# DreamWaterFound/self_commit_ORB-SLAM2

Measured on AMD Instinct MI355X. Metric: frames/s ORB extract+match (1000 feat, 640x480), higher is better.
Workload: dtype u8; 1 GPU; batch of 256 synthetic 640x480 frames per GPU (8 distinct resident batches per step, one launch set per batch), ORB extract (1000 feat, 8 levels, FAST 20/7) + brute-force Hamming SearchByBoW of consecutive frames; batch_per_gpu=256, streams=3, width=640, height=480, nfeatures=1000, parallelism=frames sharded, 1 rank(s), no data-path collective

## Files before the change

### self_commit_orb-slam2_amd/csrc/orbx_match.hip

```cpp
#include <math.h>
#include <string.h>

#include <atomic>
#include <chrono>

#include <type_traits>
#include <vector>

#include "orbx_match_internal.h"

using namespace orbx_match;

namespace {

__global__ __launch_bounds__(256) void k_bow_order(FeatDev A, const int32_t *__restrict__ pairsA, int32_t *__restrict__ order, int stride)
{
    const int p = blockIdx.y, fa = pairsA[p];
    const int nA = min(A.counts[fa], A.cap);
    const int i = blockIdx.x * 256 + threadIdx.x;
    if (i >= nA) return;
    int32_t *ord = order + (size_t)p * stride;
    if (!A.groups) { ord[i] = i; return; }
    const int32_t *g = A.groups + (size_t)fa * A.cap;
    const int gi = g[i];
// ... 387 lines not shown
    const bool act = live && !(FILTER && gA < 0);
#pragma unroll
    for (int q = 0; q < TOPK; q++) kk[q] = act ? sentinel : 0u;
    uint32_t th = kk[TOPK - 1] >> 16;
    __syncthreads();
    const unsigned char *myB = sDesc + (size_t)sl * slicePitch;
    const int j0 = sl * per, jn = max(0, min(per, nB - j0));
    for (int j = 0; j < per; j++) {
        const uint4 lo = *(const uint4 *)(myB + (size_t)j * 32), hi = *(const uint4 *)(myB + (size_t)j * 32 + 16);
        uint32_t d = bcnt_acc(a[0] ^ lo.x, 0u);
        d = bcnt_acc(a[1] ^ lo.y, d); d = bcnt_acc(a[2] ^ lo.z, d); d = bcnt_acc(a[3] ^ lo.w, d);
        d = bcnt_acc(a[4] ^ hi.x, d); d = bcnt_acc(a[5] ^ hi.y, d); d = bcnt_acc(a[6] ^ hi.z, d); d = bcnt_acc(a[7] ^ hi.w, d);
        if (FILTER) d = sG[j0 + j] == gA ? d : 0xffffu;
        const uint32_t key = (j < jn && d < th) ? (d << 16) | (uint32_t)(j0 + j) : 0xffffffffu;
        if (__any(key < kk[TOPK - 1])) { topk_insert(kk, key); th = kk[TOPK - 1] >> 16; }
    }
#pragma unroll
    for (int m = 1; m < PAIR_SLICES; m <<= 1) {
        uint32_t other[TOPK];
#pragma unroll
        for (int q = 0; q < TOPK; q++) other[q] = (uint32_t)__shfl_xor((int)kk[q], m);
#pragma unroll
        for (int q = 0; q < TOPK; q++) if (__any(other[q] < kk[TOPK - 1])) topk_insert(kk, other[q]);
    }
    if (sl == 0 && live) {
        uint4 *out = (uint4 *)(topk + (size_t)row * TOPK);
        uint32_t o[TOPK];
#pragma unroll
        for (int q = 0; q < TOPK; q++) o[q] = (!act || kk[q] >= sentinel) ? KEY_EMPTY : kk[q];
        out[0] = make_uint4(o[0], o[1], o[2], o[3]); out[1] = make_uint4(o[4], o[5], o[6], o[7]);
    }
}

#define GREEDY_THREADS 1024
__global__ __launch_bounds__(GREEDY_THREADS) void k_bow_greedy(FeatDev A, FeatDev B, const int32_t *__restrict__ pairsA, const int32_t *__restrict__ pairsB, int mode,
                                                    float nnratio, int checkOri, const uint32_t *__restrict__ topk, const int32_t *__restrict__ order,
                                                    int32_t *__restrict__ matches, int32_t *__restrict__ dists, int32_t *__restrict__ nmatches, int stride, TriDev T,
                                                    int32_t *__restrict__ pubMatches, unsigned long long *pubFlag, unsigned long long pubSeq)
{
    extern __shared__ __attribute__((aligned(16))) unsigned char smem[];
    __shared__ int hist[HISTO_LENGTH];
    __shared__ int sChangedP[2], sQueued, sTotal, sRemoved;
    const int p = blockIdx.x, tid = threadIdx.x, lane = tid & 63, wv = tid >> 6, fa = pairsA[p], fb = pairsB[p];
    const int nA = min(A.counts[fa], A.cap), nB = min(B.counts[fb], B.cap);
    uint32_t *owner = (uint32_t *)smem;
    uint32_t *dec = owner + B.cap;
    unsigned short *sOrd = (unsigned short *)(dec + A.cap);
    unsigned short *queue = sOrd + ((A.cap + 7) & ~7);
    float *sAngB = pubFlag ? (float *)(queue + ((A.cap + 7) & ~7)) : nullptr;
    int32_t *sRes = pubFlag ? (int32_t *)(sAngB + B.cap) : nullptr;
    int32_t *mout = matches + (size_t)p * stride, *dout = dists + (size_t)p * stride;
    const uint4 *tk = (const uint4 *)(topk + (size_t)p * stride * TOPK);
    const orbx_keypoint *kA = A.kp + (size_t)fa * A.cap, *kB = B.kp + (size_t)fb * B.cap;
    if (tid < HISTO_LENGTH) hist[tid] = 0;
    if (tid == 0) { sTotal = 0; sRemoved = 0; }
    float angA0 = 0.0f;
    {
        const int32_t *ord = order + (size_t)p * stride;
        for (int r = tid; r < nA; r += GREEDY_THREADS) {
            int i = ord[r];
            if (pubFlag && r == tid) angA0 = kA[i].angle;
            if (A.valid && !A.valid[(size_t)fa * A.cap + i]) i = 0xffff;
            sOrd[r] = (unsigned short)i;
            dec[r] = KEY_EMPTY;
        }
    }
    if (pubFlag) {
        for (int j = tid; j < nB; j += GREEDY_THREADS) sAngB[j] = kB[j].angle;
        const int nOut0 = mode == 0 ? nB : nA;
        for (int s2 = tid; s2 < nOut0; s2 += GREEDY_THREADS) sRes[s2] = -1;
    }
    for (int s = tid; s < stride; s += GREEDY_THREADS) { mout[s] = -1; dout[s] = 256; }
    uint4 myK0 = make_uint4(0u, 0u, 0u, 0u), myK1 = myK0, othK0 = myK0, othK1 = myK0;
    bool haveKeys = false;
    for (int j = tid; j < nB; j += GREEDY_THREADS) owner[j] = 0xffffffffu;
    if (tid == 0) { sChangedP[0] = 0; sChangedP[1] = 0; sQueued = 0; }
    for (int par = 0;; par ^= 1) {
        __syncthreads();
        for (int r = tid; r < nA; r += GREEDY_THREADS) {
            const uint32_t d = dec[r];
            if (d != KEY_EMPTY) atomicMin(&owner[d & 0xffff], (uint32_t)r);
        }
        __syncthreads();
        bool changed = false;
        for (int r = tid; r < nA; r += GREEDY_THREADS) {
            const int i = sOrd[r];
            if (i == 0xffff) continue;
            if (r != tid || !haveKeys) { const uint4 q0 = tk[i * 2], q1 = tk[i * 2 + 1]; if (r == tid) { myK0 = q0; myK1 = q1; haveKeys = true; } else { othK0 = q0; othK1 = q1; } }
            const uint4 q0 = r == tid ? myK0 : othK0, q1 = r == tid ? myK1 : othK1;
            const uint32_t keys[TOPK] = {q0.x, q0.y, q0.z, q0.w, q1.x, q1.y, q1.z, q1.w};
            auto half = [&](const int k0, uint32_t &h1, uint32_t &h2) -> int {
                uint32_t bi[4], ow[4];
#pragma unroll
                for (int k = 0; k < 4; k++) {
                    const uint32_t low = keys[k0 + k] & 0xffffu;
                    bi[k] = keys[k0 + k] == KEY_EMPTY ? 0u : (mode == 2 ? 0xffffu - low : low);
                }
#pragma unroll
                for (int k = 0; k < 4; k++) ow[k] = owner[bi[k]];
                int nf = 0;
                h1 = KEY_EMPTY; h2 = KEY_EMPTY;
#pragma unroll
                for (int k = 3; k >= 0; k--) {
                    const bool fr = keys[k0 + k] != KEY_EMPTY && ow[k] >= (uint32_t)r;
                    const uint32_t packed = (keys[k0 + k] & 0xffff0000u) | bi[k];
                    h2 = fr ? h1 : h2;
                    h1 = fr ? packed : h1;
                    nf += fr ? 1 : 0;
                }
                return nf;
            };
            uint32_t k1, k2;
            int nfree = half(0, k1, k2);
            if (nfree < 2 && (keys[4] & keys[5] & keys[6] & keys[7]) != KEY_EMPTY) {
                uint32_t j1, j2;
                const int nb = half(4, j1, j2);
                k2 = nfree == 1 ? j1 : j2;
                k1 = nfree == 1 ? k1 : j1;
                nfree += nb;
            }
            const uint32_t bestKey = k1;
            const int best2 = nfree >= 2 ? (int)(k2 >> 16) : 256;
            if (nfree < (mode == 2 ? 1 : 2) && keys[TOPK - 1] != KEY_EMPTY) { queue[atomicAdd(&sQueued, 1)] = (unsigned short)r; continue; }
            uint32_t nd = KEY_EMPTY;
            if (bestKey != KEY_EMPTY) {
                const int best1 = (int)(bestKey >> 16);
                if (mode == 2) nd = bestKey;
                else {
                    const bool pass = mode == 0 ? (best1 <= TH_LOW) : (best1 < TH_LOW);
                    if (pass && (float)best1 < nnratio * (float)best2) nd = bestKey;
                }
            }
            if (nd != dec[r]) { dec[r] = nd; changed = true; }
        }
        if (changed) sChangedP[par] = 1;
        __syncthreads();
        const int nq = sQueued;
        for (int q = wv; q < nq; q += GREEDY_THREADS / 64) {
            const int r = queue[q], i = sOrd[r];
            const unsigned long long *da = (const unsigned long long *)(A.desc + ((size_t)fa * A.cap + i) * 32);
            unsigned long long a[4] = {da[0], da[1], da[2], da[3]};
            const int gA = A.groups ? A.groups[(size_t)fa * A.cap + i] : 0;
            uint32_t k0 = KEY_EMPTY, k1 = KEY_EMPTY;
            for (int jj = lane; jj < nB; jj += 64) {
                if (owner[jj] < (uint32_t)r) continue;
                if (B.groups && B.groups[(size_t)fb * B.cap + jj] != gA) continue;
                if (mode >= 1 && B.valid && !B.valid[(size_t)fb * B.cap + jj]) continue;
                const unsigned long long *db = (const unsigned long long *)(B.desc + ((size_t)fb * B.cap + jj) * 32);
                int d = hamming256(a, db[0], db[1], db[2], db[3]);
                uint32_t kk = ((uint32_t)d << 16) | (uint32_t)jj;
                if (mode == 2) {
                    if (d > TH_LOW) continue;
                    const size_t ia = (size_t)fa * A.cap + i;
                    if (!tri_geom_ok(T, p, A.kp[ia], T.stereoA && T.stereoA[ia], B.kp[(size_t)fb * B.cap + jj], T.stereoB && T.stereoB[(size_t)fb * B.cap + jj])) continue;
                    kk = ((uint32_t)d << 16) | (0xffffu - (uint32_t)jj);
                }
                if (kk < k0) { k1 = k0; k0 = kk; } else if (kk < k1) k1 = kk;
            }
            uint32_t bestKey = wave_min(k0);
            if (k0 == bestKey) k0 = k1;
            const uint32_t second = wave_min(k0);
            uint32_t nd = KEY_EMPTY;
            if (bestKey != KEY_EMPTY) {
                const int best1 = (int)(bestKey >> 16), best2 = second != KEY_EMPTY ? (int)(second >> 16) : 256;
                if (mode == 2) nd = (bestKey & 0xffff0000u) | (0xffffu - (bestKey & 0xffffu));
                else {
                    const bool pass = mode == 0 ? (best1 <= TH_LOW) : (best1 < TH_LOW);
                    if (pass && (float)best1 < nnratio * (float)best2) nd = bestKey;
                }
            }
            if (lane == 0 && nd != dec[r]) { dec[r] = nd; sChangedP[par] = 1; }
        }
        if (nq) __syncthreads();
        const int again = sChangedP[par];
        if (!again) break;
        for (int j = tid; j < nB; j += GREEDY_THREADS) owner[j] = 0xffffffffu;
        if (tid == 0) { sChangedP[par ^ 1] = 0; sQueued = 0; }
    }
    const float factor = HISTO_LENGTH / 360.0f;
    int total = 0;
    for (int r = tid; r < nA; r += GREEDY_THREADS) {
        const uint32_t d = dec[r];
        if (d == KEY_EMPTY) continue;
        const int i = sOrd[r], bj = (int)(d & 0xffff), slot = mode == 0 ? bj : i;
        mout[slot] = mode == 0 ? i : bj; dout[slot] = (int)(d >> 16);
        if (sRes) sRes[slot] = mode == 0 ? i : bj;
        total++;
        if (checkOri) {
            float rot = ((pubFlag && r == tid) ? angA0 : kA[i].angle) - (sAngB ? sAngB[bj] : kB[bj].angle);
            if (rot < 0.0f) rot += 360.0f;
            int bin = (int)roundf(rot * factor);
            if (bin == HISTO_LENGTH) bin = 0;
            dec[r] = d | ((uint32_t)bin << 26);
            atomicAdd(&hist[bin], 1);
        }
    }
    total = wave_sum_xor(total);
    if (lane == 0 && total) atomicAdd(&sTotal, total);
    __syncthreads();
    if (checkOri) {
        int ind1, ind2, ind3;
        three_maxima_wave(hist, lane, ind1, ind2, ind3);
        int removed = 0;
        for (int r = tid; r < nA; r += GREEDY_THREADS) {
            const uint32_t d = dec[r];
            if (d == KEY_EMPTY) continue;
            const int b = (int)(d >> 26);
            if (b != ind1 && b != ind2 && b != ind3) {
                const int slot = mode == 0 ? (int)(d & 0xffff) : (int)sOrd[r];
                mout[slot] = -1; dout[slot] = 256; removed++;
                if (sRes) sRes[slot] = -1;
            }
        }
        removed = wave_sum_xor(removed);
        if (lane == 0 && removed) atomicAdd(&sRemoved, removed);
    }
    __syncthreads();
    if (tid == 0) nmatches[p] = sTotal - sRemoved;
    if (pubFlag) {
        const int nOut = mode == 0 ? nB : nA;
        for (int s2 = tid; s2 < nOut; s2 += GREEDY_THREADS) pubMatches[s2] = sRes[s2];
        if (tid == 0) pubMatches[nOut] = sTotal - sRemoved;
        orbx_publish(nullptr, pubFlag, pubSeq, 1u);
    }
}

__global__ __launch_bounds__(256) void k_stereo(FeatDev Lf, FeatDev Rf, const int32_t *__restrict__ pairsL, const int32_t *__restrict__ pairsR,
                                                const float *__restrict__ scaleFactors, float maxD, int32_t *__restrict__ bestIdx, int32_t *__restrict__ bestDist,
                                                int32_t *__restrict__ nmatches, int stride)
{
    const int p = blockIdx.y, fl = pairsL[p], fr = pairsR[p];
    const int nL = min(Lf.counts[fl], Lf.cap), nR = min(Rf.counts[fr], Rf.cap);
    const int lane = threadIdx.x & 63, iL = blockIdx.x * 4 + (threadIdx.x >> 6);
    if (iL >= nL) return;
    const orbx_keypoint kl = Lf.kp[(size_t)fl * Lf.cap + iL];
    const int row = (int)kl.y;
    const float minU = kl.x - maxD, maxU = kl.x - 0.0f;
    const unsigned long long *da = (const unsigned long long *)(Lf.desc + ((size_t)fl * Lf.cap + iL) * 32);
    unsigned long long a[4] = {da[0], da[1], da[2], da[3]};
    uint32_t best = ((uint32_t)TH_HIGH << 16);
    if (!(maxU < 0)) {
        const orbx_keypoint *kr = Rf.kp + (size_t)fr * Rf.cap;
        for (int iR = lane; iR < nR; iR += 64) {
            const orbx_keypoint k = kr[iR];
            const float r = 2.0f * scaleFactors[k.octave];
            const int maxr = (int)ceilf(k.y + r), minr = (int)floorf(k.y - r);
            if (row < minr || row > maxr) continue;
            if (k.octave < kl.octave - 1 || k.octave > kl.octave + 1) continue;
            if (!(k.x >= minU && k.x <= maxU)) continue;
            const unsigned long long *db = (const unsigned long long *)(Rf.desc + ((size_t)fr * Rf.cap + iR) * 32);
            const int d = hamming256(a, db[0], db[1], db[2], db[3]);
            const uint32_t key = ((uint32_t)d << 16) | (uint32_t)iR;
            if (d < TH_HIGH && key < best) best = key;
        }
// ... 373 lines not shown
        dist += __builtin_popcountll(x ^ y);
    }
    return dist;
}

extern "C" int orbx_matcher_create(int device, int max_features, int max_pairs, orbx_matcher **out)
{
    if (!out || max_features < 1 || max_features > 65535 || max_pairs < 1) { orbx_set_error("bad matcher arguments (1 <= max_features <= 65535)"); return ORBX_ERR_ARG; }
    *out = nullptr;
    orbx_matcher *m = new orbx_matcher();
    m->maxFeatures = max_features; m->maxPairs = max_pairs;
    int rc = m->open(device);
    hipEvent_t *const sync[] = {&m->evDep, &m->evDep2, &m->evPyr[0], &m->evPyr[1], &m->evDone[0], &m->evDone[1]};
    for (hipEvent_t *e : sync) if (!rc) rc = orbx_event_create(e, hipEventDisableTiming);
    for (int r = 0; r < MATCH_PROF_RING; r++)
        for (hipEvent_t *e : {&m->ev0[r], &m->ev1[r], &m->evMid[r]}) if (!rc) rc = orbx_event_create(e);
    const size_t S = (size_t)max_features, P = (size_t)max_pairs;
    if (rc || (rc = m->pairsA.ensure(P)) || (rc = m->pairsB.ensure(P)) || (rc = m->order.ensure(P * S)) || (rc = m->matches.ensure(P * S)) ||
        (rc = m->dists.ensure(P * S)) || (rc = m->nmatches.ensure(P)) || (rc = m->topk.ensure(P * S * TOPK)) || (rc = m->scales.ensure(128)) ||
        (rc = m->uright.ensure(P * S)) || (rc = m->depth.ensure(P * S)) || (rc = m->sad.ensure(P * S))) {
        orbx_matcher_destroy(m);
        return rc;
    }
    *out = m;
    return ORBX_OK;
}

extern "C" void orbx_matcher_destroy(orbx_matcher *m) { orbx_destroy_handle(m); }

__global__ void k_status_or(int *dst, const int *src, int first) { if (first) *dst = *src; else if (*src) atomicOr(dst, *src); }

namespace orbx_match {

int inherit_status(orbx_matcher *m, orbx_extractor *after, bool first)
{
    if (!after) return ORBX_OK;
    const int *w = orbx_extractor_status_word_internal(after);
    if (!w) return ORBX_OK;
    if (!m->producerStatus.p) {
        int rc = m->producerStatus.ensure(1);
        if (rc != ORBX_OK) return rc;
        ORBX_HIP_CHECK(hipMemsetAsync(m->producerStatus.p, 0, sizeof(int), m->stream));
    }
    hipLaunchKernelGGL(k_status_or, dim3(1), dim3(1), 0, m->stream, m->producerStatus.p, w, first ? 1 : 0);
    return ORBX_OK;
}

int check_producer_status(orbx_matcher *m)
{
    if (!m->producerStatus.p) return ORBX_OK;
    int v = 0;
    ORBX_HIP_CHECK(hipMemcpy(&v, m->producerStatus.p, sizeof(int), hipMemcpyDeviceToHost));
    if (!v) return ORBX_OK;
    ORBX_HIP_CHECK(hipMemset(m->producerStatus.p, 0, sizeof(int)));
    orbx_set_error("the extractor batch these results were computed from overflowed a device capacity (bits 0x%x: 1 = >%d FAST candidates in a level, "
                   "2 = quadtree node list, 4 = level keypoints): results are not the reference's", v, 32768);
    return ORBX_ERR_CAPACITY;
}

int prep_pairs(orbx_matcher *m, const orbx_feature_set *a, const orbx_feature_set *b, const int32_t *pa, const int32_t *pb, int npairs,
                      orbx_extractor *after)
{
    if (!m || !a || !b || !pa || !pb) { orbx_set_error("NULL argument"); return ORBX_ERR_ARG; }
    if (npairs < 1 || npairs > m->maxPairs) { orbx_set_error("npairs %d outside 1..%d", npairs, m->maxPairs); return ORBX_ERR_CAPACITY; }
    if (a->capacity > m->maxFeatures || b->capacity > m->maxFeatures || a->capacity < 1 || b->capacity < 1) {
        orbx_set_error("feature capacity %d/%d exceeds the matcher's max_features %d", a->capacity, b->capacity, m->maxFeatures);
        return ORBX_ERR_CAPACITY;
    }
    if (!a->keypoints || !a->descriptors || !a->counts || !b->keypoints || !b->descriptors || !b->counts) { orbx_set_error("NULL feature arrays"); return ORBX_ERR_ARG; }
    for (int p = 0; p < npairs; p++)
        if (pa[p] < 0 || pa[p] >= a->nframes || pb[p] < 0 || pb[p] >= b->nframes) { orbx_set_error("pair %d references a frame out of range", p); return ORBX_ERR_ARG; }
    ORBX_HIP_CHECK(hipSetDevice(m->device));
    if (after) {
        ORBX_HIP_CHECK(hipEventRecord(m->evDep, orbx_extractor_stream_internal(after)));
        ORBX_HIP_CHECK(hipStreamWaitEvent(m->stream, m->evDep, 0));
        int rcs = inherit_status(m, after, true);
        if (rcs != ORBX_OK) return rcs;
    } else if (m->producerStatus.p)
        ORBX_HIP_CHECK(hipMemsetAsync(m->producerStatus.p, 0, sizeof(int), m->stream));
    ORBX_HIP_CHECK(hipMemcpyAsync(m->pairsA.p, pa, (size_t)npairs * sizeof(int32_t), hipMemcpyHostToDevice, m->stream));
    ORBX_HIP_CHECK(hipMemcpyAsync(m->pairsB.p, pb, (size_t)npairs * sizeof(int32_t), hipMemcpyHostToDevice, m->stream));
    return ORBX_OK;
}

int chain_back(orbx_matcher *m, orbx_extractor *after)
{
    if (!after) return ORBX_OK;
    hipEvent_t ev = m->evDone[m->doneSlot];
    m->doneSlot ^= 1;
    ORBX_HIP_CHECK(hipEventRecord(ev, m->stream));
    orbx_extractor_set_consumer_event_internal(after, ev);
    return ORBX_OK;
}

FeatDev to_dev(const orbx_feature_set *s)
{
    FeatDev f;
    f.kp = s->keypoints; f.desc = s->descriptors; f.counts = s->counts; f.groups = s->groups; f.valid = s->valid; f.cap = s->capacity;
    return f;
}

}

extern "C" int orbx_search_by_bow_device(orbx_matcher *m, const orbx_feature_set *a, const orbx_feature_set *b, const int32_t *pairs_a,
                                         const int32_t *pairs_b, int npairs, const orbx_bow_params *params, orbx_extractor *after)
{
    if (!params || (params->mode != 0 && params->mode != 1)) { orbx_set_error("bad bow params"); return ORBX_ERR_ARG; }
    int rc = prep_pairs(m, a, b, pairs_a, pairs_b, npairs, after);
    if (rc != ORBX_OK) return rc;
    const int stride = m->maxFeatures;
    FeatDev A = to_dev(a), B = to_dev(b);
    const int slot = m->profCount % MATCH_PROF_RING;
    ORBX_HIP_CHECK(hipEventRecord(m->ev0[slot], m->stream));
    uint32_t dcut = TH_LOW + 1;
    while (dcut < 257 && !(params->nn_ratio * (float)dcut > (float)TH_LOW)) dcut++;
    const bool filter = b->groups != nullptr || (params->mode == 1 && b->valid != nullptr);
    const dim3 gridTopk((unsigned)((a->capacity + TOPK_ROWS - 1) / TOPK_ROWS), (unsigned)npairs);
    if (filter)
        hipLaunchKernelGGL((k_bow_topk<true, false, TOPK_NROW>), gridTopk, dim3(256), 0, m->stream, A, B, m->pairsA.p, m->pairsB.p, params->mode, dcut, m->topk.p, stride, TriDev());
    else {
        const char *em = getenv("ORBX_MATCH_MFMA");
        const bool mfma = em && em[0] == '1';
        static const int dbg = getenv("ORBX_MFMA_DEBUG") ? atoi(getenv("ORBX_MFMA_DEBUG")) : 0;
        if (mfma) hipLaunchKernelGGL(k_bow_topk_mfma, dim3((unsigned)((a->capacity + 255) / 256), (unsigned)npairs), dim3(256), 0, m->stream, A, B, m->pairsA.p, m->pairsB.p, dcut, m->topk.p, stride, dbg);
        else hipLaunchKernelGGL((k_bow_topk<false, false, TOPK_NROW>), gridTopk, dim3(256), 0, m->stream, A, B, m->pairsA.p, m->pairsB.p, params->mode, dcut, m->topk.p, stride, TriDev());
    }
    ORBX_LAUNCH_CHECK();
    ORBX_HIP_CHECK(hipEventRecord(m->evMid[slot], m->stream));
    m->midValid[slot] = true;
    hipLaunchKernelGGL(k_bow_order, dim3((unsigned)((a->capacity + 255) / 256), (unsigned)npairs), dim3(256), 0, m->stream, A, m->pairsA.p, m->order.p, stride);
    ORBX_LAUNCH_CHECK();
    const size_t ldsGreedy = (size_t)b->capacity * 4 + (size_t)a->capacity * 4 + (size_t)((a->capacity + 7) & ~7) * 2 * 2;
    if (ldsGreedy > 160 * 1024) { orbx_set_error("feature capacity %d too large for the LDS tile", a->capacity); return ORBX_ERR_CAPACITY; }
    if (ldsGreedy > 48 * 1024) ORBX_HIP_CHECK(hipFuncSetAttribute((const void *)k_bow_greedy, hipFuncAttributeMaxDynamicSharedMemorySize, (int)ldsGreedy));
    hipLaunchKernelGGL(k_bow_greedy, dim3((unsigned)npairs), dim3(GREEDY_THREADS), ldsGreedy, m->stream, A, B, m->pairsA.p, m->pairsB.p, params->mode, params->nn_ratio,
                       params->check_orientation, m->topk.p, m->order.p, m->matches.p, m->dists.p, m->nmatches.p, stride, TriDev(), (int32_t *)nullptr, (unsigned long long *)nullptr, 0ull);
    ORBX_LAUNCH_CHECK();
    ORBX_HIP_CHECK(hipEventRecord(m->ev1[slot], m->stream));
    m->profCount++;
    m->lastPairs = npairs; m->lastStride = stride;
    return chain_back(m, after);
}

extern "C" int orbx_stereo_match_device(orbx_matcher *m, const orbx_feature_set *left, const orbx_feature_set *right, const int32_t *pairs_l,
                                        const int32_t *pairs_r, int npairs, const float *scale_factors, int nlevels, float max_disparity,
                                        orbx_extractor *after)
{
    if (!scale_factors || nlevels < 1 || nlevels > 64) { orbx_set_error("bad scale factor table"); return ORBX_ERR_ARG; }
    int rc = prep_pairs(m, left, right, pairs_l, pairs_r, npairs, after);
    if (rc != ORBX_OK) return rc;
    const int stride = m->maxFeatures;
    ORBX_HIP_CHECK(hipMemcpyAsync(m->scales.p, scale_factors, (size_t)nlevels * sizeof(float), hipMemcpyHostToDevice, m->stream));
    ORBX_HIP_CHECK(hipMemsetAsync(m->nmatches.p, 0, (size_t)npairs * sizeof(int32_t), m->stream));
    const int slot = m->profCount % MATCH_PROF_RING;
    ORBX_HIP_CHECK(hipEventRecord(m->ev0[slot], m->stream));
    m->midValid[slot] = false;
    hipLaunchKernelGGL(k_stereo, dim3((unsigned)((left->capacity + 3) / 4), (unsigned)npairs), dim3(256), 0, m->stream, to_dev(left), to_dev(right), m->pairsA.p,
                       m->pairsB.p, m->scales.p, max_disparity, m->matches.p, m->dists.p, m->nmatches.p, stride);
    ORBX_LAUNCH_CHECK();
    ORBX_HIP_CHECK(hipEventRecord(m->ev1[slot], m->stream));
    m->profCount++;
    m->lastPairs = npairs; m->lastStride = stride;
    return chain_back(m, after);
}

extern "C" int orbx_compute_stereo_matches_device(orbx_matcher *m, orbx_extractor *left, orbx_extractor *right, const int32_t *frames_l,
                                                  const int32_t *frames_r, int npairs, float mbf, float mb)
{
    if (!m || !left || !right || !frames_l || !frames_r) { orbx_set_error("NULL argument"); return ORBX_ERR_ARG; }
    OrbxLastBatchView vl, vr;
// ... 321 lines not shown
    const auto sDescB = pin.add(b->descriptors, NB * 32);
    const auto sGrB = pin.add(b->groups, b->groups ? NB : 0);
    const auto sValB = pin.add(b->valid, b->valid ? NB : 0);
    const auto sCnt = pin.add(cnt, 2);
    const auto rRes = pout.hole<int32_t>((size_t)nOut + 1);
    int rc;
    const OrbxStaged sg = bx.begin(m->stream, &rc);
    if (rc != ORBX_OK) return rc;
    uint8_t *ar;
    if ((rc = orbx_stage_to_arena(bx, m->arena, m->stream, 512, &ar)) != ORBX_OK) return rc;
    ORBX_LAUNCH_CHECK();
    const int32_t *dc = sCnt.in(ar);
    FeatDev A, B;
    A.kp = sKpA.in(ar); A.desc = sDescA.in(ar); A.groups = a->groups ? sGrA.in(ar) : nullptr; A.valid = a->valid ? sValA.in(ar) : nullptr; A.counts = dc; A.cap = nA;
    B.kp = sKpB.in(ar); B.desc = sDescB.in(ar); B.groups = b->groups ? sGrB.in(ar) : nullptr; B.valid = b->valid ? sValB.in(ar) : nullptr; B.counts = dc + 1; B.cap = nB;
    uint32_t dcut = TH_LOW + 1;
    while (dcut < 257 && !(prm->nn_ratio * (float)dcut > (float)TH_LOW)) dcut++;
    const bool filter = b->groups != nullptr || (prm->mode == 1 && b->valid != nullptr);
    const int nRowBlocks = (nA + PAIR_ROWS - 1) / PAIR_ROWS, nOrder = (nA + 31) / 32;
    const int per = (nB + PAIR_SLICES - 1) / PAIR_SLICES;
    const size_t ldsPair = std::max((size_t)PAIR_SLICES * ((size_t)per * 32 + 16) + (size_t)PAIR_SLICES * per * 4, (size_t)4096 * 4);
    if ((rc = m->topk.ensure(NA * TOPK)) != ORBX_OK || (rc = m->order.ensure(NA)) != ORBX_OK) return rc;
    const dim3 grid((unsigned)(nRowBlocks + nOrder));
    if (filter) {
        if (ldsPair > 48 * 1024) ORBX_HIP_CHECK(hipFuncSetAttribute((const void *)k_bow_topk_pair<true>, hipFuncAttributeMaxDynamicSharedMemorySize, (int)ldsPair));
        hipLaunchKernelGGL(k_bow_topk_pair<true>, grid, dim3(256), ldsPair, m->stream, A, B, prm->mode, dcut, nRowBlocks, per, m->topk.p, m->order.p);
    } else {
        if (ldsPair > 48 * 1024) ORBX_HIP_CHECK(hipFuncSetAttribute((const void *)k_bow_topk_pair<false>, hipFuncAttributeMaxDynamicSharedMemorySize, (int)ldsPair));
        hipLaunchKernelGGL(k_bow_topk_pair<false>, grid, dim3(256), ldsPair, m->stream, A, B, prm->mode, dcut, nRowBlocks, per, m->topk.p, m->order.p);
    }
    ORBX_LAUNCH_CHECK();
    const size_t ldsGreedy = NB * 4 + NA * 4 + (size_t)((nA + 7) & ~7) * 2 * 2 + NB * 4 + std::max(NA, NB) * 4;
    if (ldsGreedy > 160 * 1024) { orbx_set_error("feature count %d too large for the LDS tile", nA); return ORBX_ERR_CAPACITY; }
    if (ldsGreedy > 48 * 1024) ORBX_HIP_CHECK(hipFuncSetAttribute((const void *)k_bow_greedy, hipFuncAttributeMaxDynamicSharedMemorySize, (int)ldsGreedy));
    if (!m->sfZero.p) {
        if ((rc = m->sfZero.ensure(4)) != ORBX_OK) return rc;
        ORBX_HIP_CHECK(hipMemsetAsync(m->sfZero.p, 0, 4 * sizeof(int32_t), m->stream));
    }
    const int stride = m->maxFeatures;
    const unsigned long long seq = bx.arm();
    hipLaunchKernelGGL(k_bow_greedy, dim3(1), dim3(GREEDY_THREADS), ldsGreedy, m->stream, A, B, (const int32_t *)m->sfZero.p, (const int32_t *)m->sfZero.p, prm->mode, prm->nn_ratio,
                       prm->check_orientation, m->topk.p, m->order.p, m->matches.p, m->dists.p, m->nmatches.p, stride, TriDev(), sg.dev(rRes), bx.flagDev, seq);
    ORBX_LAUNCH_CHECK();
    m->lastPairs = 1; m->lastStride = stride;
    if ((rc = bx.wait(m->stream)) != ORBX_OK) return rc;
    const int32_t *res = sg.host(rRes);
    if (nOut > 0) memcpy(matches, res, (size_t)nOut * 4);
    *nmatches = res[nOut];
    return ORBX_OK;
}

extern "C" int orbx_search_by_bow(orbx_matcher *m, const orbx_feature_set *a_host, const orbx_feature_set *b_host, const orbx_bow_params *params,
                                  int32_t *matches, int32_t *nmatches)
{
    if (!m || !matches || !nmatches) { orbx_set_error("NULL argument"); return ORBX_ERR_ARG; }
    if (!params || (params->mode != 0 && params->mode != 1)) { orbx_set_error("bad bow params"); return ORBX_ERR_ARG; }
    ORBX_HIP_CHECK(hipSetDevice(m->device));
    static const bool split = !(getenv("ORBX_BOW_SINGLE_SPLIT") && getenv("ORBX_BOW_SINGLE_SPLIT")[0] == '0');
    if (split && a_host && b_host && a_host->keypoints && a_host->descriptors && a_host->counts && b_host->keypoints && b_host->descriptors && b_host->counts &&
        a_host->counts[0] > 0 && b_host->counts[0] > 0 && a_host->counts[0] <= m->maxFeatures && b_host->counts[0] <= std::min(m->maxFeatures, 4000))
        return search_by_bow_single(m, a_host, b_host, params, matches, nmatches);
    orbx_feature_set da, db;
    const orbx_feature_set *const hostSets[2] = {a_host, b_host};
    orbx_feature_set *const devSets[2] = {&da, &db};
    int rc;
    if ((rc = stage_host(m, hostSets, devSets, 2)) != ORBX_OK) return rc;
    const int32_t zero = 0;
    if ((rc = orbx_search_by_bow_device(m, &da, &db, &zero, &zero, 1, params, nullptr)) != ORBX_OK) return rc;
    ORBX_HIP_CHECK(hipStreamSynchronize(m->stream));
    const int nOut = params->mode == 0 ? b_host->counts[0] : a_host->counts[0];
    if (nOut > 0) ORBX_HIP_CHECK(hipMemcpy(matches, m->matches.p, (size_t)nOut * 4, hipMemcpyDeviceToHost));
    ORBX_HIP_CHECK(hipMemcpy(nmatches, m->nmatches.p, 4, hipMemcpyDeviceToHost));
    return ORBX_OK;
}

extern "C" int orbx_search_for_triangulation_device(orbx_matcher *m, const orbx_feature_set *a, const orbx_feature_set *b, const int32_t *pairs_a,
                                                    const int32_t *pairs_b, int npairs, const orbx_triangulation_params *params, orbx_extractor *after)
{
    if (!params || !params->f12 || !params->epipole || !params->scale_factors || !params->level_sigma2) { orbx_set_error("bad triangulation params"); return ORBX_ERR_ARG; }
    if (params->nlevels < 1 || params->nlevels > ORBX_MAX_LEVELS) { orbx_set_error("nlevels %d outside 1..%d", params->nlevels, ORBX_MAX_LEVELS); return ORBX_ERR_ARG; }
    int rc = prep_pairs(m, a, b, pairs_a, pairs_b, npairs, after);
    if (rc != ORBX_OK) return rc;
    if ((rc = m->triGeom.ensure((size_t)11 * m->maxPairs)) != ORBX_OK) return rc;
    ORBX_HIP_CHECK(hipMemcpyAsync(m->triGeom.p, params->f12, (size_t)9 * npairs * sizeof(float), hipMemcpyHostToDevice, m->stream));
    ORBX_HIP_CHECK(hipMemcpyAsync(m->triGeom.p + (size_t)9 * m->maxPairs, params->epipole, (size_t)2 * npairs * sizeof(float), hipMemcpyHostToDevice, m->stream));
    TriDev T = TriDev();
    T.f12 = m->triGeom.p; T.epipole = m->triGeom.p + (size_t)9 * m->maxPairs;
    T.stereoA = params->stereo_a; T.stereoB = params->stereo_b;
    for (int l = 0; l < params->nlevels; l++) {
        T.epiTh[l] = 100 * params->scale_factors[l];
        T.chiTh[l] = 3.84 * params->level_sigma2[l];
    }
    const int stride = m->maxFeatures;
    FeatDev A = to_dev(a), B = to_dev(b);
    const int slot = m->profCount % MATCH_PROF_RING;
    ORBX_HIP_CHECK(hipEventRecord(m->ev0[slot], m->stream));
    hipLaunchKernelGGL(k_bow_order, dim3((unsigned)((a->capacity + 255) / 256), (unsigned)npairs), dim3(256), 0, m->stream, A, m->pairsA.p, m->order.p, stride);
    ORBX_LAUNCH_CHECK();
    const dim3 gridTopk((unsigned)((a->capacity + TOPK_ROWS - 1) / TOPK_ROWS), (unsigned)npairs);
    hipLaunchKernelGGL((k_bow_topk<true, true, TOPK_NROW>), gridTopk, dim3(256), 0, m->stream, A, B, m->pairsA.p, m->pairsB.p, 2, (uint32_t)(TH_LOW + 1), m->topk.p, stride, T);
    ORBX_LAUNCH_CHECK();
    m->midValid[slot] = false;
    const size_t ldsGreedy = (size_t)b->capacity * 4 + (size_t)a->capacity * 4 + (size_t)((a->capacity + 7) & ~7) * 2 * 2;
    if (ldsGreedy > 160 * 1024) { orbx_set_error("feature capacity %d too large for the LDS tile", a->capacity); return ORBX_ERR_CAPACITY; }
    if (ldsGreedy > 48 * 1024) ORBX_HIP_CHECK(hipFuncSetAttribute((const void *)k_bow_greedy, hipFuncAttributeMaxDynamicSharedMemorySize, (int)ldsGreedy));
    hipLaunchKernelGGL(k_bow_greedy, dim3((unsigned)npairs), dim3(GREEDY_THREADS), ldsGreedy, m->stream, A, B, m->pairsA.p, m->pairsB.p, 2, 0.0f, params->check_orientation,
                       m->topk.p, m->order.p, m->matches.p, m->dists.p, m->nmatches.p, stride, T, (int32_t *)nullptr, (unsigned long long *)nullptr, 0ull);
    ORBX_LAUNCH_CHECK();
    ORBX_HIP_CHECK(hipEventRecord(m->ev1[slot], m->stream));
    m->profCount++;
    m->lastPairs = npairs; m->lastStride = stride;
    return chain_back(m, after);
}

extern "C" int orbx_search_for_triangulation(orbx_matcher *m, const orbx_feature_set *a_host, const orbx_feature_set *b_host,
                                             const orbx_triangulation_params *params_host, int32_t *matches12, int32_t *nmatches)
{
    if (!m || !params_host || !matches12 || !nmatches) { orbx_set_error("NULL argument"); return ORBX_ERR_ARG; }
    ORBX_HIP_CHECK(hipSetDevice(m->device));
    orbx_feature_set da, db;
    const orbx_feature_set *const hostSets[2] = {a_host, b_host};
    orbx_feature_set *const devSets[2] = {&da, &db};
    int rc;
    if ((rc = stage_host(m, hostSets, devSets, 2)) != ORBX_OK) return rc;
    orbx_triangulation_params P = *params_host;
    const uint8_t *hostFlags[2] = {params_host->stereo_a, params_host->stereo_b};
    const int cnt[2] = {a_host->counts[0], b_host->counts[0]};
    const uint8_t *devFlags[2] = {nullptr, nullptr};
    for (int sd = 0; sd < 2; sd++) {
        if (!hostFlags[sd]) continue;
        if ((rc = m->hs[sd].ensure((size_t)m->maxFeatures)) != ORBX_OK) return rc;
        if (cnt[sd] > 0) ORBX_HIP_CHECK(hipMemcpyAsync(m->hs[sd].p, hostFlags[sd], (size_t)cnt[sd], hipMemcpyHostToDevice, m->stream));
        devFlags[sd] = m->hs[sd].p;
    }
    P.stereo_a = devFlags[0]; P.stereo_b = devFlags[1];
    const int32_t zero = 0;
    if ((rc = orbx_search_for_triangulation_device(m, &da, &db, &zero, &zero, 1, &P, nullptr)) != ORBX_OK) return rc;
    ORBX_HIP_CHECK(hipStreamSynchronize(m->stream));
    if (cnt[0] > 0) ORBX_HIP_CHECK(hipMemcpy(matches12, m->matches.p, (size_t)cnt[0] * 4, hipMemcpyDeviceToHost));
    ORBX_HIP_CHECK(hipMemcpy(nmatches, m->nmatches.p, 4, hipMemcpyDeviceToHost));
    return ORBX_OK;
// ... 23 lines not shown
```

### self_commit_orb-slam2_amd/csrc/orbx_match_internal.h

```cpp
#ifndef ORBX_MATCH_INTERNAL_H
#define ORBX_MATCH_INTERNAL_H

#include "orbx_handle.h"
#include <vector>

#define TH_HIGH 100
#define TH_LOW 50
#define HISTO_LENGTH 30
#define KEY_EMPTY 0xffffffffu
#define TOPK 8
#define MATCH_PROF_RING 64

#define KEY64_EMPTY 0xffffffffffffffffull
#define GRID_COLS 64
#define GRID_ROWS 48

struct FeatDev {
    const orbx_keypoint *kp;
    const uint8_t *desc;
    const int32_t *counts;
    const int32_t *groups;
    const uint8_t *valid;
    int cap;
};
// ... 6 lines not shown

__device__ __forceinline__ void three_maxima_wave(const int *hist, int lane, int &ind1, int &ind2, int &ind3)
{
    const int c = lane < HISTO_LENGTH ? hist[lane] : 0;
    uint32_t key = c > 0 ? ((uint32_t)c << 5) | (uint32_t)(31 - lane) : 0u;
    uint32_t top[3];
#pragma unroll
    for (int k = 0; k < 3; k++) {
        uint32_t v = key;
#pragma unroll
        for (int o = 32; o > 0; o >>= 1) { const uint32_t u = __shfl_xor(v, o); v = u > v ? u : v; }
        top[k] = v;
        if (key == v) key = 0u;
    }
    const int max1 = (int)(top[0] >> 5), max2 = (int)(top[1] >> 5), max3 = (int)(top[2] >> 5);
    ind1 = top[0] ? 31 - (int)(top[0] & 31u) : -1; ind2 = top[1] ? 31 - (int)(top[1] & 31u) : -1; ind3 = top[2] ? 31 - (int)(top[2] & 31u) : -1;
    if ((float)max2 < 0.1f * (float)max1) { ind2 = -1; ind3 = -1; }
    else if ((float)max3 < 0.1f * (float)max1) { ind3 = -1; }
}

struct ProjFrameDev { const orbx_keypoint *kp; const uint8_t *desc; const float *uRight; const uint8_t *occupied; const int32_t *counts; int cap;
                      float minX, minY, gwInv, ghInv; };

struct orbx_matcher : OrbxHandle {
    int maxFeatures = 0, maxPairs = 0;
    hipEvent_t evDep = nullptr, evDone[2] = {nullptr, nullptr};
    int doneSlot = 0;
    hipEvent_t ev0[MATCH_PROF_RING] = {}, ev1[MATCH_PROF_RING] = {};
    hipEvent_t evMid[MATCH_PROF_RING] = {};
    bool midValid[MATCH_PROF_RING] = {};
    float lastDistanceMs = 0.f, lastReplayMs = 0.f;
    int profCount = 0;
    OrbxOwnedBuf<int32_t> pairsA, pairsB, order, matches, dists, nmatches;
    OrbxOwnedBuf<uint32_t> topk;
    OrbxOwnedBuf<float> scales, uright, depth, pf[2];
    OrbxOwnedBuf<unsigned long long> topk64;
    OrbxOwnedBuf<uint8_t> pb[2];
    OrbxOwnedBuf<int32_t> pi32[2];
    OrbxOwnedBuf<orbx_keypoint> pkp;
    OrbxOwnedBuf<uint32_t> projDec, projQueue;
    OrbxHostStage hostStage;
    OrbxCallBox box;
    OrbxOwnedBuf<uint8_t> arena;
    OrbxOwnedBuf<int32_t> sad;
    OrbxOwnedBuf<int32_t> stRowStart, stRowList;
    hipEvent_t evDep2 = nullptr, evPyr[2] = {nullptr, nullptr};
    int lastStereoPairs = 0;
    float sfScales[128] = {};
    int sfLevels = 0;
    OrbxOwnedBuf<int32_t> sfZero;
    OrbxOwnedBuf<float> sfScalesDev;
    float *sfHost = nullptr, *sfHostDev = nullptr;
    size_t sfHostFloats = 0;
    int sfSeq = 0, sfFlagSeq = 0;
    int sfPending = 0;
    OrbxOwnedBuf<orbx_keypoint> hk[2];
    OrbxOwnedBuf<uint8_t> hd[2], hv[2];
    OrbxOwnedBuf<int32_t> hc[2], hg[2];
    OrbxOwnedBuf<uint8_t> hs[2];
    OrbxOwnedBuf<float> triGeom;
    OrbxOwnedBuf<float> frProj;
    OrbxOwnedBuf<int32_t> frLevel;
    OrbxOwnedBuf<uint8_t> frInView;
    size_t frCount = 0;
    int lastPairs = 0, lastStride = 0;
    OrbxOwnedBuf<int> producerStatus;
// ... 41 lines not shown
                if (gamma != 0.0) {
                    const double zeta = (beta - alpha) / (2.0 * gamma);
                    const double t = copysign(1.0, zeta) / (fabs(zeta) + sqrt(1.0 + zeta * zeta));
                    c = 1.0 / sqrt(1.0 + t * t);
                    s = c * t;
                }
#pragma unroll
                for (int r = 0; r < 4; r++) {
                    const double ap = a[p][r], aq = a[q][r];
                    a[p][r] = c * ap - s * aq;
                    a[q][r] = s * ap + c * aq;
                    const double vp = v[p][r], vq = v[q][r];
                    v[p][r] = c * vp - s * vq;
                    v[q][r] = s * vp + c * vq;
                }
            }
        }
    }
    double best = 0.0;
#pragma unroll
    for (int c = 0; c < 4; c++) {
        double n2 = 0.0;
#pragma unroll
        for (int r = 0; r < 4; r++) n2 = n2 + a[c][r] * a[c][r];
        const bool take = c == 0 || n2 < best;
        best = take ? n2 : best;
#pragma unroll
        for (int r = 0; r < 4; r++) nv[r] = take ? v[c][r] : nv[r];
    }
}
#endif

namespace orbx_match {
int prep_pairs(orbx_matcher *m, const orbx_feature_set *a, const orbx_feature_set *b, const int32_t *pa, const int32_t *pb, int npairs, orbx_extractor *after);
int chain_back(orbx_matcher *m, orbx_extractor *after);
int inherit_status(orbx_matcher *m, orbx_extractor *after, bool first = true);
int check_producer_status(orbx_matcher *m);
FeatDev to_dev(const orbx_feature_set *s);
int stage_host(orbx_matcher *m, const orbx_feature_set *const *h, orbx_feature_set *const *d, int nsides);
}

#endif
```

Before: 316,900 frames/s.

## Cut BoW matcher launch overhead and keep replay top-k keys in registers

```diff
diff --git a/self_commit_orb-slam2_amd/csrc/orbx_match.hip b/self_commit_orb-slam2_amd/csrc/orbx_match.hip
--- a/self_commit_orb-slam2_amd/csrc/orbx_match.hip
+++ b/self_commit_orb-slam2_amd/csrc/orbx_match.hip
@@ -443,12 +443,16 @@
     }
 }
 
-#define GREEDY_THREADS 1024
-__global__ __launch_bounds__(GREEDY_THREADS) void k_bow_greedy(FeatDev A, FeatDev B, const int32_t *__restrict__ pairsA, const int32_t *__restrict__ pairsB, int mode,
+#define REPLAY_REG_RANKS 1024
+template <int THREADS>
+__global__ __launch_bounds__(THREADS) void k_bow_greedy(FeatDev A, FeatDev B, const int32_t *__restrict__ pairsA, const int32_t *__restrict__ pairsB, int mode,
                                                     float nnratio, int checkOri, const uint32_t *__restrict__ topk, const int32_t *__restrict__ order,
                                                     int32_t *__restrict__ matches, int32_t *__restrict__ dists, int32_t *__restrict__ nmatches, int stride, TriDev T,
-                                                    int32_t *__restrict__ pubMatches, unsigned long long *pubFlag, unsigned long long pubSeq)
-{
+                                                    int32_t *__restrict__ pubMatches, unsigned long long *pubFlag, unsigned long long pubSeq,
+                                                    int *statusDst, const int *statusSrc)
+{
+    static_assert(THREADS >= 64 && THREADS % 64 == 0 && THREADS <= 1024, "whole waves; the histogram is cleared by the first HISTO_LENGTH threads");
+    constexpr int RPT = (REPLAY_REG_RANKS + THREADS - 1) / THREADS;
     extern __shared__ __attribute__((aligned(16))) unsigned char smem[];
     __shared__ int hist[HISTO_LENGTH];
     __shared__ int sChangedP[2], sQueued, sTotal, sRemoved;
@@ -465,40 +469,47 @@
     const orbx_keypoint *kA = A.kp + (size_t)fa * A.cap, *kB = B.kp + (size_t)fb * B.cap;
     if (tid < HISTO_LENGTH) hist[tid] = 0;
     if (tid == 0) { sTotal = 0; sRemoved = 0; }
+    if (statusDst && p == 0 && tid == 0) *statusDst = *statusSrc;
     float angA0 = 0.0f;
+    uint4 myK0[RPT], myK1[RPT];
     {
-        const int32_t *ord = order + (size_t)p * stride;
-        for (int r = tid; r < nA; r += GREEDY_THREADS) {
-            int i = ord[r];
+        const int32_t *ord = order ? order + (size_t)p * stride : nullptr;
+        auto initRank = [&](const int r) -> int {
+            int i = ord ? ord[r] : r;
             if (pubFlag && r == tid) angA0 = kA[i].angle;
             if (A.valid && !A.valid[(size_t)fa * A.cap + i]) i = 0xffff;
             sOrd[r] = (unsigned short)i;
             dec[r] = KEY_EMPTY;
-        }
+            return i;
+        };
+#pragma unroll
+        for (int s = 0; s < RPT; s++) {
+            myK0[s] = make_uint4(0u, 0u, 0u, 0u); myK1[s] = myK0[s];
+            const int r = tid + s * THREADS;
+            if (r < nA) {
+                const int i = initRank(r);
+                if (i != 0xffff) { myK0[s] = tk[i * 2]; myK1[s] = tk[i * 2 + 1]; }
+            }
+        }
+        for (int r = tid + RPT * THREADS; r < nA; r += THREADS) initRank(r);
     }
     if (pubFlag) {
-        for (int j = tid; j < nB; j += GREEDY_THREADS) sAngB[j] = kB[j].angle;
+        for (int j = tid; j < nB; j += THREADS) sAngB[j] = kB[j].angle;
         const int nOut0 = mode == 0 ? nB : nA;
-        for (int s2 = tid; s2 < nOut0; s2 += GREEDY_THREADS) sRes[s2] = -1;
-    }
-    for (int s = tid; s < stride; s += GREEDY_THREADS) { mout[s] = -1; dout[s] = 256; }
-    uint4 myK0 = make_uint4(0u, 0u, 0u, 0u), myK1 = myK0, othK0 = myK0, othK1 = myK0;
-    bool haveKeys = false;
-    for (int j = tid; j < nB; j += GREEDY_THREADS) owner[j] = 0xffffffffu;
+        for (int s2 = tid; s2 < nOut0; s2 += THREADS) sRes[s2] = -1;
+    }
+    for (int s = tid; s < stride; s += THREADS) { mout[s] = -1; dout[s] = 256; }
+    for (int j = tid; j < nB; j += THREADS) owner[j] = 0xffffffffu;
     if (tid == 0) { sChangedP[0] = 0; sChangedP[1] = 0; sQueued = 0; }
     for (int par = 0;; par ^= 1) {
         __syncthreads();
-        for (int r = tid; r < nA; r += GREEDY_THREADS) {
+        for (int r = tid; r < nA; r += THREADS) {
             const uint32_t d = dec[r];
             if (d != KEY_EMPTY) atomicMin(&owner[d & 0xffff], (uint32_t)r);
         }
         __syncthreads();
         bool changed = false;
-        for (int r = tid; r < nA; r += GREEDY_THREADS) {
-            const int i = sOrd[r];
-            if (i == 0xffff) continue;
-            if (r != tid || !haveKeys) { const uint4 q0 = tk[i * 2], q1 = tk[i * 2 + 1]; if (r == tid) { myK0 = q0; myK1 = q1; haveKeys = true; } else { othK0 = q0; othK1 = q1; } }
-            const uint4 q0 = r == tid ? myK0 : othK0, q1 = r == tid ? myK1 : othK1;
+        auto decide = [&](const int r, const uint4 q0, const uint4 q1) {
             const uint32_t keys[TOPK] = {q0.x, q0.y, q0.z, q0.w, q1.x, q1.y, q1.z, q1.w};
             auto half = [&](const int k0, uint32_t &h1, uint32_t &h2) -> int {
                 uint32_t bi[4], ow[4];
@@ -532,7 +543,7 @@
             }
             const uint32_t bestKey = k1;
             const int best2 = nfree >= 2 ? (int)(k2 >> 16) : 256;
-            if (nfree < (mode == 2 ? 1 : 2) && keys[TOPK - 1] != KEY_EMPTY) { queue[atomicAdd(&sQueued, 1)] = (unsigned short)r; continue; }
+            if (nfree < (mode == 2 ? 1 : 2) && keys[TOPK - 1] != KEY_EMPTY) { queue[atomicAdd(&sQueued, 1)] = (unsigned short)r; return; }
             uint32_t nd = KEY_EMPTY;
             if (bestKey != KEY_EMPTY) {
                 const int best1 = (int)(bestKey >> 16);
@@ -543,11 +554,20 @@
                 }
             }
             if (nd != dec[r]) { dec[r] = nd; changed = true; }
+        };
+#pragma unroll
+        for (int s = 0; s < RPT; s++) {
+            const int r = tid + s * THREADS;
+            if (r < nA && sOrd[r] != 0xffff) decide(r, myK0[s], myK1[s]);
+        }
+        for (int r = tid + RPT * THREADS; r < nA; r += THREADS) {
+            const int i = sOrd[r];
+            if (i != 0xffff) decide(r, tk[i * 2], tk[i * 2 + 1]);
         }
         if (changed) sChangedP[par] = 1;
         __syncthreads();
         const int nq = sQueued;
-        for (int q = wv; q < nq; q += GREEDY_THREADS / 64) {
+        for (int q = wv; q < nq; q += THREADS / 64) {
             const int r = queue[q], i = sOrd[r];
             const unsigned long long *da = (const unsigned long long *)(A.desc + ((size_t)fa * A.cap + i) * 32);
             unsigned long long a[4] = {da[0], da[1], da[2], da[3]};
@@ -585,12 +605,12 @@
         if (nq) __syncthreads();
         const int again = sChangedP[par];
         if (!again) break;
-        for (int j = tid; j < nB; j += GREEDY_THREADS) owner[j] = 0xffffffffu;
+        for (int j = tid; j < nB; j += THREADS) owner[j] = 0xffffffffu;
         if (tid == 0) { sChangedP[par ^ 1] = 0; sQueued = 0; }
     }
     const float factor = HISTO_LENGTH / 360.0f;
     int total = 0;
-    for (int r = tid; r < nA; r += GREEDY_THREADS) {
+    for (int r = tid; r < nA; r += THREADS) {
         const uint32_t d = dec[r];
         if (d == KEY_EMPTY) continue;
         const int i = sOrd[r], bj = (int)(d & 0xffff), slot = mode == 0 ? bj : i;
@@ -613,7 +633,7 @@
         int ind1, ind2, ind3;
         three_maxima_wave(hist, lane, ind1, ind2, ind3);
         int removed = 0;
-        for (int r = tid; r < nA; r += GREEDY_THREADS) {
+        for (int r = tid; r < nA; r += THREADS) {
             const uint32_t d = dec[r];
             if (d == KEY_EMPTY) continue;
             const int b = (int)(d >> 26);
@@ -630,7 +650,7 @@
     if (tid == 0) nmatches[p] = sTotal - sRemoved;
     if (pubFlag) {
         const int nOut = mode == 0 ? nB : nA;
-        for (int s2 = tid; s2 < nOut; s2 += GREEDY_THREADS) pubMatches[s2] = sRes[s2];
+        for (int s2 = tid; s2 < nOut; s2 += THREADS) pubMatches[s2] = sRes[s2];
         if (tid == 0) pubMatches[nOut] = sTotal - sRemoved;
         orbx_publish(nullptr, pubFlag, pubSeq, 1u);
     }
@@ -1070,7 +1090,7 @@
 
 namespace orbx_match {
 
-int inherit_status(orbx_matcher *m, orbx_extractor *after, bool first)
+int inherit_status(orbx_matcher *m, orbx_extractor *after, bool first, const int **defer)
 {
     if (!after) return ORBX_OK;
     const int *w = orbx_extractor_status_word_internal(after);
@@ -1080,6 +1100,7 @@
         if (rc != ORBX_OK) return rc;
         ORBX_HIP_CHECK(hipMemsetAsync(m->producerStatus.p, 0, sizeof(int), m->stream));
     }
+    if (defer) { *defer = w; return ORBX_OK; }
     hipLaunchKernelGGL(k_status_or, dim3(1), dim3(1), 0, m->stream, m->producerStatus.p, w, first ? 1 : 0);
     return ORBX_OK;
 }
@@ -1097,8 +1118,9 @@
 }
 
 int prep_pairs(orbx_matcher *m, const orbx_feature_set *a, const orbx_feature_set *b, const int32_t *pa, const int32_t *pb, int npairs,
-                      orbx_extractor *after)
-{
+                      orbx_extractor *after, const int **deferStatus)
+{
+    if (deferStatus) *deferStatus = nullptr;
     if (!m || !a || !b || !pa || !pb) { orbx_set_error("NULL argument"); return ORBX_ERR_ARG; }
     if (npairs < 1 || npairs > m->maxPairs) { orbx_set_error("npairs %d outside 1..%d", npairs, m->maxPairs); return ORBX_ERR_CAPACITY; }
     if (a->capacity > m->maxFeatures || b->capacity > m->maxFeatures || a->capacity < 1 || b->capacity < 1) {
@@ -1109,15 +1131,23 @@
     for (int p = 0; p < npairs; p++)
         if (pa[p] < 0 || pa[p] >= a->nframes || pb[p] < 0 || pb[p] >= b->nframes) { orbx_set_error("pair %d references a frame out of range", p); return ORBX_ERR_ARG; }
     ORBX_HIP_CHECK(hipSetDevice(m->device));
+    std::vector<int32_t> &h = m->pairsHost;
+    const size_t bytes = (size_t)npairs * sizeof(int32_t);
+    if (!(npairs <= m->pairsHostN && !memcmp(h.data(), pa, bytes) && !memcmp(h.data() + m->pairsHostN, pb, bytes))) {
+        m->pairsHostN = 0;
+        ORBX_HIP_CHECK(hipMemcpyAsync(m->pairsA.p, pa, bytes, hipMemcpyHostToDevice, m->stream));
+        ORBX_HIP_CHECK(hipMemcpyAsync(m->pairsB.p, pb, bytes, hipMemcpyHostToDevice, m->stream));
+        h.assign(pa, pa + npairs);
+        h.insert(h.end(), pb, pb + npairs);
+        m->pairsHostN = npairs;
+    }
     if (after) {
         ORBX_HIP_CHECK(hipEventRecord(m->evDep, orbx_extractor_stream_internal(after)));
         ORBX_HIP_CHECK(hipStreamWaitEvent(m->stream, m->evDep, 0));
-        int rcs = inherit_status(m, after, true);
+        int rcs = inherit_status(m, after, true, deferStatus);
         if (rcs != ORBX_OK) return rcs;
     } else if (m->producerStatus.p)
         ORBX_HIP_CHECK(hipMemsetAsync(m->producerStatus.p, 0, sizeof(int), m->stream));
-    ORBX_HIP_CHECK(hipMemcpyAsync(m->pairsA.p, pa, (size_t)npairs * sizeof(int32_t), hipMemcpyHostToDevice, m->stream));
-    ORBX_HIP_CHECK(hipMemcpyAsync(m->pairsB.p, pb, (size_t)npairs * sizeof(int32_t), hipMemcpyHostToDevice, m->stream));
     return ORBX_OK;
 }
 
@@ -1140,11 +1170,28 @@
 
 }
 
+template <typename... Args>
+static int launch_bow_replay(orbx_matcher *m, int npairs, size_t lds, Args... args)
+{
+    int threads = 1024;
+    if (const char *e = getenv("ORBX_BOW_REPLAY_THREADS")) {
+        const int v = atoi(e);
+        if (v == 256 || v == 512 || v == 1024) threads = v;
+    }
+    auto *k = threads == 256 ? &k_bow_greedy<256> : threads == 512 ? &k_bow_greedy<512> : &k_bow_greedy<1024>;
+    if (lds > 160 * 1024) { orbx_set_error("feature capacity too large for the replay's LDS tile (%zu bytes)", lds); return ORBX_ERR_CAPACITY; }
+    if (lds > 48 * 1024) ORBX_HIP_CHECK(hipFuncSetAttribute((const void *)k, hipFuncAttributeMaxDynamicSharedMemorySize, (int)lds));
+    hipLaunchKernelGGL(k, dim3((unsigned)npairs), dim3((unsigned)threads), lds, m->stream, args...);
+    ORBX_LAUNCH_CHECK();
+    return ORBX_OK;
+}
+
 extern "C" int orbx_search_by_bow_device(orbx_matcher *m, const orbx_feature_set *a, const orbx_feature_set *b, const int32_t *pairs_a,
                                          const int32_t *pairs_b, int npairs, const orbx_bow_params *params, orbx_extractor *after)
 {
     if (!params || (params->mode != 0 && params->mode != 1)) { orbx_set_error("bad bow params"); return ORBX_ERR_ARG; }
-    int rc = prep_pairs(m, a, b, pairs_a, pairs_b, npairs, after);
+    const int *statusSrc = nullptr;
+    int rc = prep_pairs(m, a, b, pairs_a, pairs_b, npairs, after, &statusSrc);
     if (rc != ORBX_OK) return rc;
     const int stride = m->maxFeatures;
     FeatDev A = to_dev(a), B = to_dev(b);
@@ -1166,14 +1213,17 @@
     ORBX_LAUNCH_CHECK();
     ORBX_HIP_CHECK(hipEventRecord(m->evMid[slot], m->stream));
     m->midValid[slot] = true;
-    hipLaunchKernelGGL(k_bow_order, dim3((unsigned)((a->capacity + 255) / 256), (unsigned)npairs), dim3(256), 0, m->stream, A, m->pairsA.p, m->order.p, stride);
-    ORBX_LAUNCH_CHECK();
+    const int32_t *order = nullptr;
+    if (A.groups) {
+        hipLaunchKernelGGL(k_bow_order, dim3((unsigned)((a->capacity + 255) / 256), (unsigned)npairs), dim3(256), 0, m->stream, A, m->pairsA.p, m->order.p, stride);
+        ORBX_LAUNCH_CHECK();
+        order = m->order.p;
+    }
     const size_t ldsGreedy = (size_t)b->capacity * 4 + (size_t)a->capacity * 4 + (size_t)((a->capacity + 7) & ~7) * 2 * 2;
-    if (ldsGreedy > 160 * 1024) { orbx_set_error("feature capacity %d too large for the LDS tile", a->capacity); return ORBX_ERR_CAPACITY; }
-    if (ldsGreedy > 48 * 1024) ORBX_HIP_CHECK(hipFuncSetAttribute((const void *)k_bow_greedy, hipFuncAttributeMaxDynamicSharedMemorySize, (int)ldsGreedy));
-    hipLaunchKernelGGL(k_bow_greedy, dim3((unsigned)npairs), dim3(GREEDY_THREADS), ldsGreedy, m->stream, A, B, m->pairsA.p, m->pairsB.p, params->mode, params->nn_ratio,
-                       params->check_orientation, m->topk.p, m->order.p, m->matches.p, m->dists.p, m->nmatches.p, stride, TriDev(), (int32_t *)nullptr, (unsigned long long *)nullptr, 0ull);
-    ORBX_LAUNCH_CHECK();
+    if ((rc = launch_bow_replay(m, npairs, ldsGreedy, A, B, m->pairsA.p, m->pairsB.p, params->mode, params->nn_ratio, params->check_orientation, m->topk.p, order,
+                                m->matches.p, m->dists.p, m->nmatches.p, stride, TriDev(), (int32_t *)nullptr, (unsigned long long *)nullptr, 0ull,
+                                statusSrc ? m->producerStatus.p : (int *)nullptr, statusSrc)) != ORBX_OK)
+        return rc;
     ORBX_HIP_CHECK(hipEventRecord(m->ev1[slot], m->stream));
     m->profCount++;
     m->lastPairs = npairs; m->lastStride = stride;
@@ -1561,16 +1611,16 @@
     ORBX_LAUNCH_CHECK();
     const size_t ldsGreedy = NB * 4 + NA * 4 + (size_t)((nA + 7) & ~7) * 2 * 2 + NB * 4 + std::max(NA, NB) * 4;
     if (ldsGreedy > 160 * 1024) { orbx_set_error("feature count %d too large for the LDS tile", nA); return ORBX_ERR_CAPACITY; }
-    if (ldsGreedy > 48 * 1024) ORBX_HIP_CHECK(hipFuncSetAttribute((const void *)k_bow_greedy, hipFuncAttributeMaxDynamicSharedMemorySize, (int)ldsGreedy));
     if (!m->sfZero.p) {
         if ((rc = m->sfZero.ensure(4)) != ORBX_OK) return rc;
         ORBX_HIP_CHECK(hipMemsetAsync(m->sfZero.p, 0, 4 * sizeof(int32_t), m->stream));
     }
     const int stride = m->maxFeatures;
     const unsigned long long seq = bx.arm();
-    hipLaunchKernelGGL(k_bow_greedy, dim3(1), dim3(GREEDY_THREADS), ldsGreedy, m->stream, A, B, (const int32_t *)m->sfZero.p, (const int32_t *)m->sfZero.p, prm->mode, prm->nn_ratio,
-                       prm->check_orientation, m->topk.p, m->order.p, m->matches.p, m->dists.p, m->nmatches.p, stride, TriDev(), sg.dev(rRes), bx.flagDev, seq);
-    ORBX_LAUNCH_CHECK();
+    if ((rc = launch_bow_replay(m, 1, ldsGreedy, A, B, (const int32_t *)m->sfZero.p, (const int32_t *)m->sfZero.p, prm->mode, prm->nn_ratio, prm->check_orientation,
+                                m->topk.p, (const int32_t *)m->order.p, m->matches.p, m->dists.p, m->nmatches.p, stride, TriDev(), sg.dev(rRes), bx.flagDev, seq, (int *)nullptr,
+                                (const int *)nullptr)) != ORBX_OK)
+        return rc;
     m->lastPairs = 1; m->lastStride = stride;
     if ((rc = bx.wait(m->stream)) != ORBX_OK) return rc;
     const int32_t *res = sg.host(rRes);
@@ -1631,11 +1681,10 @@
     ORBX_LAUNCH_CHECK();
     m->midValid[slot] = false;
     const size_t ldsGreedy = (size_t)b->capacity * 4 + (size_t)a->capacity * 4 + (size_t)((a->capacity + 7) & ~7) * 2 * 2;
-    if (ldsGreedy > 160 * 1024) { orbx_set_error("feature capacity %d too large for the LDS tile", a->capacity); return ORBX_ERR_CAPACITY; }
-    if (ldsGreedy > 48 * 1024) ORBX_HIP_CHECK(hipFuncSetAttribute((const void *)k_bow_greedy, hipFuncAttributeMaxDynamicSharedMemorySize, (int)ldsGreedy));
-    hipLaunchKernelGGL(k_bow_greedy, dim3((unsigned)npairs), dim3(GREEDY_THREADS), ldsGreedy, m->stream, A, B, m->pairsA.p, m->pairsB.p, 2, 0.0f, params->check_orientation,
-                       m->topk.p, m->order.p, m->matches.p, m->dists.p, m->nmatches.p, stride, T, (int32_t *)nullptr, (unsigned long long *)nullptr, 0ull);
-    ORBX_LAUNCH_CHECK();
+    if ((rc = launch_bow_replay(m, npairs, ldsGreedy, A, B, m->pairsA.p, m->pairsB.p, 2, 0.0f, params->check_orientation, m->topk.p, (const int32_t *)m->order.p,
+                                m->matches.p, m->dists.p, m->nmatches.p, stride, T, (int32_t *)nullptr, (unsigned long long *)nullptr, 0ull, (int *)nullptr,
+                                (const int *)nullptr)) != ORBX_OK)
+        return rc;
     ORBX_HIP_CHECK(hipEventRecord(m->ev1[slot], m->stream));
     m->profCount++;
     m->lastPairs = npairs; m->lastStride = stride;
diff --git a/self_commit_orb-slam2_amd/csrc/orbx_match_internal.h b/self_commit_orb-slam2_amd/csrc/orbx_match_internal.h
--- a/self_commit_orb-slam2_amd/csrc/orbx_match_internal.h
+++ b/self_commit_orb-slam2_amd/csrc/orbx_match_internal.h
@@ -62,6 +62,8 @@
     float lastDistanceMs = 0.f, lastReplayMs = 0.f;
     int profCount = 0;
     OrbxOwnedBuf<int32_t> pairsA, pairsB, order, matches, dists, nmatches;
+    std::vector<int32_t> pairsHost;
+    int pairsHostN = 0;
     OrbxOwnedBuf<uint32_t> topk;
     OrbxOwnedBuf<float> scales, uright, depth, pf[2];
     OrbxOwnedBuf<unsigned long long> topk64;
@@ -169,9 +171,10 @@
 #endif
 
 namespace orbx_match {
-int prep_pairs(orbx_matcher *m, const orbx_feature_set *a, const orbx_feature_set *b, const int32_t *pa, const int32_t *pb, int npairs, orbx_extractor *after);
+int prep_pairs(orbx_matcher *m, const orbx_feature_set *a, const orbx_feature_set *b, const int32_t *pa, const int32_t *pb, int npairs, orbx_extractor *after,
+               const int **deferStatus = nullptr);
 int chain_back(orbx_matcher *m, orbx_extractor *after);
-int inherit_status(orbx_matcher *m, orbx_extractor *after, bool first = true);
+int inherit_status(orbx_matcher *m, orbx_extractor *after, bool first = true, const int **defer = nullptr);
 int check_producer_status(orbx_matcher *m);
 FeatDev to_dev(const orbx_feature_set *s);
 int stage_host(orbx_matcher *m, const orbx_feature_set *const *h, orbx_feature_set *const *d, int nsides);
```

Result: no change. 316,500 frames/s (-0.1%).
